# mitsuba-renderer/enoki

Measured on AMD Instinct MI355X. Metric: Gelem/s + %HBM-roofline, 64M-elt DiffArray backward(), 1/2/4/8 MI355X, higher is better.
Workload: dtype f32; 1 GPU; cfg3b: DiffArray<HIPArray<float>> y=hsum(sin(a*x+b)), a=gather(A,idx), b=gather(B,idx), K=1Mi; backward() with scatter_add grads; elements_total=67108864, elements_per_gpu=67108864, table_size=1048576, world_size=1, backend=none (single process), step_replay=eager (python-driven steps: tape walk, allocator, one launch call per kernel)

## Files before the change

enoki_amd/csrc/bucketed_early.hip:

```cpp
#include "ek_bucketed.h"
#include "ek_refine.h"

#include <cstdlib>
#include <cstring>

namespace ek {

template <int Map, int Keep, typename T> struct EarlyPair {
    static __device__ __forceinline__ void apply(T u, T &val, T &kept) {
        if constexpr ((Map == EK_SIN && Keep == EK_COS) || (Map == EK_COS && Keep == EK_SIN)) {
            T sn, cs;
            SinCosOp::apply(u, sn, cs);
            val = Map == EK_SIN ? sn : cs;
            kept = Map == EK_SIN ? cs : sn;
        } else if constexpr (Map == Keep) {
            val = kept = UnaryOp<Map, T>::apply(u);
        } else {
            val = UnaryOp<Map, T>::apply(u);
            kept = UnaryOp<Keep, T>::apply(u);
        }
    }
};

#ifdef EK_EARLY_TIMING
__device__ unsigned long long g_early_timing[32];
#endif

template <typename T, int V, int Map, int Keep, bool Two>
struct EarlyBody {
    static constexpr bool Paired = sizeof(T) == 4;
    struct Step { Pack<uint16_t, 4> pi[V]; T px[V][4]; };
    const PairRec<T> *rec;
    T *tables;
    unsigned long long *dummy;
    const uint16_t *pair_idx;
    const T *x_b;
    int Bins;
    uint32_t lmask;
    T acc[4];
#ifdef EK_EARLY_TIMING
    unsigned long long tacc[5] = { 0, 0, 0, 0, 0 }, tlast = 0, tmark[2] = { 0, 0 };
    __device__ __forceinline__ void mark(int k) { tmark[k] = __builtin_readcyclecounter(); }
    __device__ __forceinline__ void stamp(int k) { const unsigned long long now = __builtin_readcyclecounter(); tacc[k] += now - tlast; tlast = now; }
#endif

    __device__ __forceinline__ void values(uint32_t l, T x, T &sum, T &v0, T &v1) const {
        const PairRec<T> r = rec[l];
        EarlyPair<Map, Keep, T>::apply(pair_value(r.a, x, r.c, Two), sum, v0);
        v1 = dev::safe_mul(x, v0);
    }
    __device__ __forceinline__ void one(size_t pos, bool on, int slot) {
        const uint32_t l = on ? (uint32_t) pair_idx[pos] & lmask : 0u;
        T sum, v0, v1;
        values(l, on ? x_b[pos] : T(0), sum, v0, v1);
        if (on) acc[slot] += sum;
        if constexpr (Paired) {
            lds_add_pair(reinterpret_cast<unsigned long long *>(tables) + l, v0, v1, on);
        } else {
            lds_add<true>(&tables[l], v0, on);
            lds_add<true>(&tables[Bins + l], v1, on);
        }
    }
    __device__ __forceinline__ void fetch(Step &s, int h, size_t pos) {
        s.pi[h] = pack_load<uint16_t, 4, true>(pair_idx + pos);
        load4<T, true>(x_b + pos, s.px[h]);
    }
    __device__ __forceinline__ void apply(const Step &s) {
        constexpr int NB = 4 * V;
        uint32_t l[NB];
        T v0[NB], v1[NB];
        if constexpr (Paired) {
            unsigned long long *tb = reinterpret_cast<unsigned long long *>(tables);
            PairRec<T> r[NB];
#ifdef EK_EARLY_TIMING
            tlast = __builtin_readcyclecounter();
            asm volatile("s_waitcnt vmcnt(3)" ::: "memory");
            stamp(0);
#endif
#pragma unroll
            for (int k = 0; k < NB; ++k) {
                l[k] = (uint32_t) s.pi[k / 4].v[k % 4] & lmask;
                r[k] = rec[l[k]];
            }
#ifdef EK_EARLY_TIMING
            asm volatile("s_waitcnt lgkmcnt(0)" ::: "memory");
            stamp(1);
#endif
            unsigned pending = 0;
#pragma unroll
            for (int k = 0; k < NB; ++k) {
                const T x = s.px[k / 4][k % 4];
                T sum;
                EarlyPair<Map, Keep, T>::apply(pair_value(r[k].a, x, r[k].c, Two), sum, v0[k]);
                v1[k] = dev::safe_mul(x, v0[k]);
                acc[k % 4] += sum;
                pending |= lds_try_add_pair(tb, dummy, l[k], v0[k], v1[k]) ? 1u << k : 0u;
            }
#ifdef EK_EARLY_TIMING
            asm volatile("s_waitcnt lgkmcnt(0)" ::: "memory");
            stamp(2);
#endif
            if (__builtin_amdgcn_ballot_w64(pending != 0)) lds_add_pair_retry<NB>(tb, l, v0, v1, pending);
#ifdef EK_EARLY_TIMING
            asm volatile("s_waitcnt lgkmcnt(0)" ::: "memory");
            stamp(3);
            tacc[4] += 1;
#endif
            return;
        }
#pragma unroll
        for (int k = 0; k < NB; ++k) {
            l[k] = (uint32_t) s.pi[k / 4].v[k % 4] & lmask;
            T sum;
            values(l[k], s.px[k / 4][k % 4], sum, v0[k], v1[k]);
            acc[k % 4] += sum;
        }
        if constexpr (!Paired) {
            lds_add_batch<T, NB>(tables, l, v0);
            lds_add_batch<T, NB>(tables + Bins, l, v1);
        }
    }
};



__device__ __forceinline__ unsigned long long to_fixed64(float v, double up) {
    const double d = __builtin_fma((double) v, up, 6755399441055744.0);
    return __builtin_bit_cast(unsigned long long, d) - 0x4338000000000000ull;
}

constexpr uint32_t kFixedRecBytes = 4096u * 8u;

template <int PS, int Map, int Keep, bool Two>
struct EarlyFixed {
    using T = float;
    static constexpr uint32_t Page = 1u << PS, LX = Page / 4, PW = 64 / LX;
    struct Step { Pack<uint16_t, 4> pi; T px[4]; };
    const unsigned char *lds;
    const uint16_t *pair_idx;
    const T *x_b;
    uint32_t m8;
    double up0, up1;
    long long iacc;

    __device__ __forceinline__ void fetch(Step &s, size_t pos) {
#ifdef EK_FX_DIAG_IDXPAIR
        const uint32_t lane = threadIdx.x & 63u, even = (lane / (2 * LX)) * 2 * LX + lane % LX;
        const uint32_t page = (uint32_t) (pos >> PS), pa = (uint32_t) __shfl((int) page, (int) even, 64);
        const size_t posl = ((size_t) (pa & ~1u) << PS) + (((lane / LX) & 1u) << PS) + (pos & (Page - 1u));
        s.pi = pack_load<uint16_t, 4, true>(pair_idx + posl);
#else
        s.pi = pack_load<uint16_t, 4, true>(pair_idx + pos);
#endif
        load4<T, true>(x_b + pos, s.px);
    }
    struct Recs { uint32_t a8[4]; PairRec<T> r[4]; };
    __device__ __forceinline__ void lookup(const Step &s, Recs &o) const {
        uint32_t w[2];
        __builtin_memcpy(w, &s.pi, 8);
        o.a8[0] = (w[0] << 3) & m8; o.a8[1] = (w[0] >> 13) & m8;
        o.a8[2] = (w[1] << 3) & m8; o.a8[3] = (w[1] >> 13) & m8;
#pragma unroll
        for (int k = 0; k < 4; ++k) o.r[k] = *reinterpret_cast<const PairRec<T> *>(lds + o.a8[k]);
#ifdef EK_FX_DIAG_NOLOOKUP
#pragma unroll
        for (int k = 0; k < 4; ++k) o.r[k] = PairRec<T>{ __uint_as_float(o.a8[k] | 0x3f000000u), T(0.25) };
#endif
    }
    template <bool Masked>
    __device__ __forceinline__ void apply(const Step &s, const Recs &rc, int rem) {
        const uint32_t *a8 = rc.a8;
        const PairRec<T> *r = rc.r;
        int batch = 0;
#pragma unroll
        for (int k = 0; k < 4; ++k) {
            const T x = s.px[k];
            const T u = pair_value(r[k].a, x, r[k].c, Two);
            T sn = T(0), cs = T(0);
#ifdef EK_FX_DIAG_NOSINCOS
            sn = u; cs = u * T(0.5);
#else
            dev::sincos_f32<Map == EK_SIN || Keep == EK_SIN, Map == EK_COS || Keep == EK_COS, true>(u, sn, cs);
#endif
            const T sum = Map == EK_SIN ? sn : cs;
            T v0 = Keep == EK_SIN ? sn : cs;
            int q = dev::cvt_sat_i32(sum * 268435456.0f);
            if constexpr (Masked) {
                const bool on = k < rem;
                q = on ? q : 0;
                v0 = on ? v0 : T(0);
            }
            batch += q;
            const T v1 = dev::safe_mul(x, v0);
            unsigned long long *p = reinterpret_cast<unsigned long long *>(const_cast<unsigned char *>(lds) + kFixedRecBytes + a8[k]);
            unsigned long long *p1 = reinterpret_cast<unsigned long long *>(const_cast<unsigned char *>(lds) + 2 * kFixedRecBytes + a8[k]);
#ifdef EK_FX_DIAG_NOADDS
            batch += (int) (to_fixed64(v0, up0) >> 20) + (int) (to_fixed64(v1, up1) >> 20) + (int) (size_t) p;
#else
            (void) __hip_atomic_fetch_add(p, to_fixed64(v0, up0), __ATOMIC_RELAXED, __HIP_MEMORY_SCOPE_WORKGROUP);
            (void) __hip_atomic_fetch_add(p1, to_fixed64(v1, up1), __ATOMIC_RELAXED, __HIP_MEMORY_SCOPE_WORKGROUP);
#endif
        }
        iacc += (long long) batch;
    }
    __device__ __forceinline__ void flush() { }
};

template <int PS, typename Body>
__device__ __forceinline__ void walk_pages_dynamic(const BucketLists &bl, const PieceRange &r, Body &body, uint32_t *s_next) {
    using Step = typename Body::Step;
    constexpr uint32_t LX = Body::LX, PW = Body::PW, Page = Body::Page;
    const uint32_t lane = threadIdx.x & 63u, gw = lane / LX, i = lane % LX, wave = threadIdx.x >> 6;
    const uint32_t nfull = r.f1 - r.f0, nparts = r.p1 - r.p0, total = nfull + nparts, nb = (total + PW - 1u) / PW;
    auto grab = [&]() -> uint32_t {
        uint32_t v = 0;
        if (lane == 0) v = __hip_atomic_fetch_add(s_next, 1u, __ATOMIC_RELAXED, __HIP_MEMORY_SCOPE_WORKGROUP);
        return v;
    };
    auto entry = [&](uint32_t b) -> uint32_t {
        const uint32_t q = b * PW + gw;
        const uint32_t *a = q < nfull ? bl.glist_full + r.f0 + q : q < total ? bl.glist_part + r.p0 + (q - nfull) : bl.base;
        return __builtin_nontemporal_load(a);
    };
    auto place = [&](uint32_t b, uint32_t ev, size_t &pos, int &rem) {
        const uint32_t q = b * PW + gw;
        const uint32_t page = q < nfull ? ev : q < total ? ev >> 6 : 0u;
        const uint32_t count = q < nfull ? Page : q < total ? (ev & 63u) + 1u : 0u;
        pos = ((size_t) page << PS) + 4u * i;
        rem = (int) count - (int) (4u * i);
    };
    uint32_t id0 = wave, id1 = wave + kBucketWaves, id2 = wave + 2 * kBucketWaves, id3 = wave + 3 * kBucketWaves, id4 = wave + 4 * kBucketWaves;
    if (id0 >= nb) return;
    uint32_t evA = entry(id0), evB = entry(id1);
    const uint32_t ev2 = entry(id2);
    Step st0, st1, st2, st3;
    typename Body::Recs r0, r1;
    size_t pos;
    int rem0, rem1, rem2, rem3 = 0;
    place(id0, evA, pos, rem0);
    body.fetch(st0, pos);
    place(id1, evB, pos, rem1);
    body.fetch(st1, pos);
    evB = entry(id3);
    place(id2, ev2, pos, rem2);
    body.fetch(st2, pos);
    body.lookup(st0, r0);
    auto phase = [&](const Step &cur, const Step &next, Step &last, const typename Body::Recs &rc, typename Body::Recs &rn, int remc, int &reml,
                     uint32_t &ev_new, uint32_t ev_old) -> bool {
        const uint32_t g5 = grab();
        ev_new = entry(id4);
        place(id3, ev_old, pos, reml);
        body.fetch(last, pos);
        body.lookup(next, rn);
        if (__builtin_amdgcn_ballot_w64(remc < 4)) body.template apply<true>(cur, rc, remc);
        else body.template apply<false>(cur, rc, 4);
        id0 = id1; id1 = id2; id2 = id3; id3 = id4; id4 = (uint32_t) __builtin_amdgcn_readfirstlane((int) g5);
        return id0 < nb;
    };
    while (true) {
        if (!phase(st0, st1, st3, r0, r1, rem0, rem3, evA, evB)) break;
        if (!phase(st1, st2, st0, r1, r0, rem1, rem0, evB, evA)) break;
        if (!phase(st2, st3, st1, r0, r1, rem2, rem1, evA, evB)) break;
        if (!phase(st3, st0, st2, r1, r0, rem3, rem2, evB, evA)) break;
    }
    body.flush();
}


struct RefinedStream {
    const float *x;
    const uint16_t *hdr;
    const uint32_t *tiles;
    uint32_t cap_tiles;
};
struct NoRefinedStream { };
template <bool Refined> using RefinedArg = std::conditional_t<Refined, RefinedStream, NoRefinedStream>;

template <int Map, int Keep, bool Two>
struct EarlyRefined {
    using T = float;
    struct Step { uint32_t h; T px[4]; };
    struct Recs { uint32_t a8; PairRec<T> r; };
    const unsigned char *lds;
    uint32_t m8;
    double up0, up1;
    long long iacc;

    __device__ __forceinline__ void lookup(const Step &s, Recs &o) const {
        o.a8 = (s.h << 3) & m8;
        o.r = *reinterpret_cast<const PairRec<T> *>(lds + o.a8);
    }
    __device__ __forceinline__ void apply(const Step &s, const Recs &rc) {
        const int count = (int) (s.h >> kRefineEntryBits);
        int batch = 0;
        unsigned long long s0 = 0ull, s1 = 0ull;
#pragma unroll
        for (int k = 0; k < 4; ++k) {
            const T x = s.px[k];
            const T u = pair_value(rc.r.a, x, rc.r.c, Two);
            T sn = T(0), cs = T(0);
            dev::sincos_f32<Map == EK_SIN || Keep == EK_SIN, Map == EK_COS || Keep == EK_COS, true>(u, sn, cs);
            const T sum = Map == EK_SIN ? sn : cs;
            T v0 = Keep == EK_SIN ? sn : cs;
            int q = dev::cvt_sat_i32(sum * 268435456.0f);
            const bool on = k < count;
            q = on ? q : 0;
            v0 = on ? v0 : T(0);
            batch += q;
            const T v1 = dev::safe_mul(x, v0);
            s0 += to_fixed64(v0, up0);
            s1 += to_fixed64(v1, up1);
        }
        unsigned long long *p = reinterpret_cast<unsigned long long *>(const_cast<unsigned char *>(lds) + kFixedRecBytes + rc.a8);
        unsigned long long *p1 = reinterpret_cast<unsigned long long *>(const_cast<unsigned char *>(lds) + 2 * kFixedRecBytes + rc.a8);
        (void) __hip_atomic_fetch_add(p, s0, __ATOMIC_RELAXED, __HIP_MEMORY_SCOPE_WORKGROUP);
        (void) __hip_atomic_fetch_add(p1, s1, __ATOMIC_RELAXED, __HIP_MEMORY_SCOPE_WORKGROUP);
        iacc += (long long) batch;
    }
};

template <typename Body>
__device__ __forceinline__ void walk_tiles_dynamic(const RefinedStream &rs, uint32_t t0, uint32_t t1, Body &body, uint32_t *s_next) {
    using Step = typename Body::Step;
    constexpr uint32_t R = kRefineR;
    static_assert(R % 4 == 0);
    const uint32_t lane = threadIdx.x & 63u, wave = threadIdx.x >> 6, nt = t1 - t0;
    uint32_t tile0 = wave, tile1 = wave + kBucketWaves;
    if (tile0 >= nt) return;
    auto fetch = [&](Step &s, uint32_t tile, uint32_t g) {
        const size_t slot = ((size_t) (t0 + tile) * R + g) * 64u + lane;
        s.h = (uint32_t) __builtin_nontemporal_load(rs.hdr + slot);
        load4<float, true>(rs.x + slot * 4u, s.px);
    };
    Step st0, st1, st2, st3;
    typename Body::Recs r0, r1;
    fetch(st0, tile0, 0);
    fetch(st1, tile0, 1);
    fetch(st2, tile0, 2);
    body.lookup(st0, r0);
    while (true) {
        uint32_t g2 = 0;
        if (lane == 0) g2 = __hip_atomic_fetch_add(s_next, 1u, __ATOMIC_RELAXED, __HIP_MEMORY_SCOPE_WORKGROUP);
        const uint32_t tnext = tile1 < nt ? tile1 : tile0;
        auto phase = [&](uint32_t g, const Step &cur, const Step &next, Step &last, const typename Body::Recs &rc, typename Body::Recs &rn) {
            const uint32_t gf = g + 3u;
            fetch(last, gf < R ? tile0 : tnext, gf & (R - 1u));
            body.lookup(next, rn);
            body.apply(cur, rc);
        };
        for (uint32_t g = 0; g < R; g += 4) {
            phase(g, st0, st1, st3, r0, r1);
            phase(g + 1, st1, st2, st0, r1, r0);
            phase(g + 2, st2, st3, st1, r0, r1);
            phase(g + 3, st3, st0, st2, r1, r0);
        }
        tile0 = tile1;
        tile1 = (uint32_t) __builtin_amdgcn_readfirstlane((int) g2);
        if (tile0 >= nt) break;
    }
}

__device__ __forceinline__ void bucket_finish_fixed_begin(long long iblock , float fblock , float *__restrict__ partials,
                                                          uint32_t *__restrict__ ticket, uint32_t *s_last_fixed ) {
    unsigned long long *ipartials = reinterpret_cast<unsigned long long *>(partials);
    uint32_t *fpartials = reinterpret_cast<uint32_t *>(ipartials + gridDim.x);
    if (threadIdx.x == 0) {
        __hip_atomic_store(ipartials + blockIdx.x, (unsigned long long) iblock, __ATOMIC_RELAXED, __HIP_MEMORY_SCOPE_AGENT);
        __hip_atomic_store(fpartials + blockIdx.x, __float_as_uint(fblock), __ATOMIC_RELAXED, __HIP_MEMORY_SCOPE_AGENT);
#ifdef EK_EARLY_TIMING
        const unsigned long long t_tk = __builtin_readcyclecounter();
#endif
        *s_last_fixed = finish_ticket(ticket) ? 1u : 0u;
#ifdef EK_EARLY_TIMING
        const unsigned long long dt_tk = __builtin_readcyclecounter() - t_tk;
        atomicAdd(&g_early_timing[24], dt_tk); atomicMax(&g_early_timing[25], dt_tk);
#endif
    }
}
__device__ __forceinline__ void bucket_finish_fixed_end(const uint32_t *s_last_fixed , float *__restrict__ partials,
                                                        uint32_t *__restrict__ ticket, float *__restrict__ out, const uint32_t *__restrict__ active,
                                                        size_t n, int map_op, float *wave_part, long long *wave_ipart, uint32_t *__restrict__ counters,
                                                        float zero_u) {
    unsigned long long *ipartials = reinterpret_cast<unsigned long long *>(partials);
    uint32_t *fpartials = reinterpret_cast<uint32_t *>(ipartials + gridDim.x);
    __syncthreads();
    if (!*s_last_fixed) return;
    if (counters) {
        for (unsigned k = threadIdx.x; k < kPgTotalsWords + 4u; k += blockDim.x) counters[k] = 0u;
        for (unsigned k = kPgMetaBase + kPgMetaAccumRep + threadIdx.x; k < kPgMetaBase + kPgMetaAccumRepEnd; k += blockDim.x) counters[k] = 0u;
    }
    long long iv = 0;
    float fv = 0.f;
    for (unsigned i = threadIdx.x; i < gridDim.x; i += blockDim.x) {
        iv += (long long) __hip_atomic_load(ipartials + i, __ATOMIC_RELAXED, __HIP_MEMORY_SCOPE_AGENT);
        fv += __uint_as_float(__hip_atomic_load(fpartials + i, __ATOMIC_RELAXED, __HIP_MEMORY_SCOPE_AGENT));
    }
#pragma unroll
    for (int d = 32; d >= 1; d >>= 1) { iv += bucket_shfl_down(iv, d); fv += bucket_shfl_down(fv, d); }
    __syncthreads();
    if ((threadIdx.x & 63) == 0) { wave_ipart[threadIdx.x >> 6] = iv; wave_part[threadIdx.x >> 6] = fv; }
    __syncthreads();
    if (threadIdx.x < 64) {
        iv = threadIdx.x < blockDim.x / 64 ? wave_ipart[threadIdx.x] : 0ll;
        fv = threadIdx.x < blockDim.x / 64 ? wave_part[threadIdx.x] : 0.f;
#pragma unroll
        for (int d = 8; d >= 1; d >>= 1) { iv += bucket_shfl_down(iv, d); fv += bucket_shfl_down(fv, d); }
        if (threadIdx.x == 0) {
            const float r = (float) iv * 3.7252902984619140625e-9f  + fv;
            out[0] = bucket_dropped_lanes<float, EK_HSUM>(r, active ? n - (size_t) active[0] : 0, active && active[1], map_op, zero_u);
            finish_ticket_reset(ticket);
        }
    }
}

template <typename T, int V, int PS, bool Fixed, bool Two, bool Refined>
__device__ __forceinline__ void bucket_pair_forward_adjoint(T *__restrict__ partials, T *__restrict__ table_partials,
                                                            const T *__restrict__ table_a, const T *__restrict__ table_c, const T addend,
                                                            size_t table_size, int flip_a, int flip_c,
                                                            const uint16_t *__restrict__ pair_idx, const T *__restrict__ x_b,
                                                            const BucketLists &bl, int map_op, int keep_op, int shift,
                                                            const BucketFinish<T> &fin, const int zero_op, const T zero_u,
                                                            const uint32_t *__restrict__ xmax_bits, int S0,
                                                            uint32_t *__restrict__ piece_mode, const RefinedArg<Refined> &refined,
                                                            T *__restrict__ direct1) {
    static_assert(!Refined || (Fixed && sizeof(T) == 4), "the refined stream feeds the fixed-point walk only");
    extern __shared__ __align__(16) unsigned char lds_dynamic[];
    __shared__ __align__(16) unsigned char lds_static[Fixed ? 3 * kFixedRecBytes : 16];
    unsigned char *lds_raw = Fixed ? lds_static : lds_dynamic;
    const int Bins = 1 << shift;
    PairRec<T> *rec = reinterpret_cast<PairRec<T> *>(lds_raw);
    T *tables = Fixed ? reinterpret_cast<T *>(lds_raw + kFixedRecBytes) : reinterpret_cast<T *>(rec + Bins);
    __shared__ T wave_part[kBucketWaves];
    __shared__ unsigned long long s_dummy;
    __shared__ uint32_t s_next;
    __shared__ uint32_t s_guard[2];
    __shared__ long long wave_ipart[Fixed ? kBucketWaves : 1];
    __shared__ uint32_t s_last_fixed;
    constexpr bool Paired = sizeof(T) == 4;
    int bucket;
    PieceRange range;
#ifdef EK_EARLY_TIMING
    const unsigned long long t_entry = __builtin_readcyclecounter();
#endif
    [[maybe_unused]] uint32_t xm_early = 0, tile_first = 0, tile_end = 0;
    if constexpr (Refined) {
        tile_first = min(refined.tiles[blockIdx.x], refined.cap_tiles);
        tile_end = min(refined.tiles[blockIdx.x + 1], refined.cap_tiles);
    }
    if constexpr (Fixed) {
        xm_early = xmax_bits[0];
        if (threadIdx.x == 0) { s_next = (Refined ? 2u : 5u) * kBucketWaves; s_guard[0] = 0u; s_guard[1] = 0u; }
    }
    if (!bucket_piece<PS>(bl, bucket, range)) {
        if constexpr (Fixed) {
            bucket_finish_fixed_begin(0ll, T(0), partials, fin.ticket, &s_last_fixed);
            bucket_finish_fixed_end(&s_last_fixed, partials, fin.ticket, fin.out, fin.active, fin.n, zero_op, wave_part, wave_ipart, fin.counters, zero_u);
        }
        else bucket_finish<T, EK_HSUM>(T(0), partials, fin.ticket, fin.out, fin.active, fin.n, zero_op, wave_part, fin.counters, zero_u);
        return;
    }
#ifdef EK_EARLY_TIMING
    const unsigned long long t_piece = __builtin_readcyclecounter();
#endif
#ifdef EK_EARLY_TIMING
    unsigned long long fx_t[6] = { 0, 0, 0, 0, 0, 0 };
    fx_t[0] = __builtin_readcyclecounter();
#endif
    [[maybe_unused]] uint32_t slice_max[2] = { 0u, 0u };
    stage_pair_slice<T, true>(rec, tables, table_a, table_c, addend, (size_t) bucket * Bins, table_size, Bins, flip_a, flip_c, Fixed ? slice_max : nullptr);
    if constexpr (Fixed) {
        for (int j = threadIdx.x; j < 2 * 4096; j += kBucketThreads) reinterpret_cast<unsigned long long *>(tables)[j] = 0ull;
    }
    if constexpr (Fixed) {
        uint32_t am = slice_max[0], cm = slice_max[1];
#pragma unroll
        for (int d = 32; d >= 1; d >>= 1) { am = max(am, (uint32_t) __shfl_xor((int) am, d, 64)); cm = max(cm, (uint32_t) __shfl_xor((int) cm, d, 64)); }
        if ((threadIdx.x & 63) == 0) { atomicMax(&s_guard[0], am); atomicMax(&s_guard[1], cm); }
    }
    __syncthreads();
    T v = T(0);
#ifdef EK_EARLY_TIMING
    unsigned long long t_walk_end = 0;
#endif
    auto run = [&](auto body) {
        body.rec = rec; body.tables = tables; body.pair_idx = pair_idx; body.x_b = x_b; body.Bins = Bins;
        body.lmask = (uint32_t) Bins - 1u; body.dummy = &s_dummy;
#pragma unroll
        for (int k = 0; k < 4; ++k) body.acc[k] = T(0);
#ifdef EK_EARLY_TIMING
        const unsigned long long t_begin = __builtin_readcyclecounter();
#endif
        walk_piece<PS, V>(bl, range, body);
#ifdef EK_EARLY_TIMING
        if ((threadIdx.x & 255) == 0) {
            const unsigned long long t_end = __builtin_readcyclecounter();
            for (int k = 0; k < 5; ++k) atomicAdd(&g_early_timing[k], body.tacc[k]);
            atomicAdd(&g_early_timing[5], t_end - t_begin);
            atomicAdd(&g_early_timing[6], 1ull);
            atomicAdd(&g_early_timing[7], body.tmark[0] - t_begin);
            atomicAdd(&g_early_timing[8], body.tmark[1] - body.tmark[0]);
            atomicAdd(&g_early_timing[9], t_end - body.tmark[1]);
            atomicAdd(&g_early_timing[10], t_piece - t_entry);
            atomicAdd(&g_early_timing[11], t_begin - t_piece);
            atomicMax(&g_early_timing[12], t_end - t_begin);
            t_walk_end = t_end;
        }
#endif
        v = (body.acc[0] + body.acc[1]) + (body.acc[2] + body.acc[3]);
    };
    [[maybe_unused]] bool locks = !Fixed, single = false;
    [[maybe_unused]] long long iv = 0;
    [[maybe_unused]] FixedScale fixed0{}, fixed1{};
    if constexpr (Fixed) {
        const uint32_t xm = (uint32_t) __builtin_amdgcn_readfirstlane((int) xm_early);
        const uint32_t E = xm >> 23;
        locks = E >= 255u || (E < (uint32_t) S0 + 1u && xm != 0u);
        const uint32_t am = s_guard[0], cm = s_guard[1];
        const float ubound = __uint_as_float(am) * __uint_as_float(xm) + __uint_as_float(cm);
        const size_t piece_pages = (size_t) (range.f1 - range.f0) + (range.p1 - range.p0);
        if (am >= 0x7F800000u || cm >= 0x7F800000u || !(ubound < 1.0e18f) || (piece_pages << PS) >> (62 - S0)) locks = true;
        single = range.pieces == 1u;
        if (threadIdx.x == 0) piece_mode[blockIdx.x] = (locks || single) ? 1u : 0u;
        if (!locks) {
            fixed0 = fixed_scale(S0, xm, false);
            fixed1 = fixed_scale(S0, xm, true);
            auto run_fixed = [&](auto body) {
                body.lds = lds_raw; body.pair_idx = pair_idx; body.x_b = x_b;
                asm volatile("v_mov_b32 %0, %1" : "=v"(body.m8) : "s"(((uint32_t) Bins - 1u) << 3));
                body.up0 = fixed0.upd; body.up1 = fixed1.upd; body.iacc = 0;
#ifdef EK_EARLY_TIMING
                fx_t[1] = __builtin_readcyclecounter();
#endif
                walk_pages_dynamic<PS>(bl, range, body, &s_next);
#ifdef EK_EARLY_TIMING
                fx_t[2] = __builtin_readcyclecounter();
#endif
                iv = body.iacc;
            };
            [[maybe_unused]] auto run_refined = [&](auto body) {
                if constexpr (Refined) {
                    body.lds = lds_raw;
                    asm volatile("v_mov_b32 %0, %1" : "=v"(body.m8) : "s"(((uint32_t) Bins - 1u) << 3));
                    body.up0 = fixed0.upd; body.up1 = fixed1.upd; body.iacc = 0;
                    walk_tiles_dynamic(refined, (uint32_t) __builtin_amdgcn_readfirstlane((int) tile_first),
                                       (uint32_t) __builtin_amdgcn_readfirstlane((int) tile_end), body, &s_next);
                    iv = body.iacc;
                }
            };
            if constexpr (Refined) {
                if (map_op == EK_SIN && keep_op == EK_COS) run_refined(EarlyRefined<EK_SIN, EK_COS, Two>{});
                else if (map_op == EK_COS && keep_op == EK_SIN) run_refined(EarlyRefined<EK_COS, EK_SIN, Two>{});
                else if (map_op == EK_SIN) run_refined(EarlyRefined<EK_SIN, EK_SIN, Two>{});
                else run_refined(EarlyRefined<EK_COS, EK_COS, Two>{});
            } else
            if (map_op == EK_SIN && keep_op == EK_COS) run_fixed(EarlyFixed<PS, EK_SIN, EK_COS, Two>{});
            else if (map_op == EK_COS && keep_op == EK_SIN) run_fixed(EarlyFixed<PS, EK_COS, EK_SIN, Two>{});
            else if (map_op == EK_SIN) run_fixed(EarlyFixed<PS, EK_SIN, EK_SIN, Two>{});
            else run_fixed(EarlyFixed<PS, EK_COS, EK_COS, Two>{});
        }
    }
    if (locks) {
#define EK_EARLY_CASE(M, K) else if (map_op == M && keep_op == K) run(EarlyBody<T, V, M, K, Two>{});
        if (map_op == EK_SIN && keep_op == EK_COS) run(EarlyBody<T, V, EK_SIN, EK_COS, Two>{});
        EK_EARLY_CASE(EK_COS, EK_SIN) EK_EARLY_CASE(EK_LOG, EK_RCP) EK_EARLY_CASE(EK_SQRT, EK_RSQRT) EK_EARLY_CASE(EK_RCP, EK_RCP_SQR)
        EK_EARLY_CASE(EK_RSQRT, EK_RSQRT_CUBE) EK_EARLY_CASE(EK_SIN, EK_SIN) EK_EARLY_CASE(EK_COS, EK_COS)
        EK_EARLY_CASE(EK_EXP, EK_EXP) EK_EARLY_CASE(EK_SQRT, EK_SQRT) EK_EARLY_CASE(EK_RCP, EK_RCP) EK_EARLY_CASE(EK_RSQRT, EK_RSQRT)
        EK_EARLY_CASE(EK_LOG, EK_LOG) EK_EARLY_CASE(EK_ABS, EK_ABS) EK_EARLY_CASE(EK_NEG, EK_NEG)
#undef EK_EARLY_CASE
    }
#pragma unroll
    for (int d = 32; d >= 1; d >>= 1) v += bucket_shfl_down(v, d);
    const int lane = threadIdx.x & 63, wave = threadIdx.x >> 6;
    if constexpr (Fixed) {
#pragma unroll
        for (int d = 32; d >= 1; d >>= 1) iv += bucket_shfl_down(iv, d);
        if (lane == 0) wave_ipart[wave] = iv;
    }
    if (lane == 0) wave_part[wave] = v;
    __syncthreads();
#ifdef EK_EARLY_TIMING
    fx_t[3] = __builtin_readcyclecounter();
#endif
    if (threadIdx.x < 64) {
        v = threadIdx.x < kBucketWaves ? wave_part[threadIdx.x] : T(0);
#pragma unroll
        for (int d = 8; d >= 1; d >>= 1) v += bucket_shfl_down(v, d);
        if constexpr (Fixed) {
            iv = threadIdx.x < kBucketWaves ? wave_ipart[threadIdx.x] : 0ll;
#pragma unroll
            for (int d = 8; d >= 1; d >>= 1) iv += bucket_shfl_down(iv, d);
        }
    }
    if constexpr (Fixed) bucket_finish_fixed_begin(iv, v, partials, fin.ticket, &s_last_fixed);
    [[maybe_unused]] bool direct = false;
    if constexpr (Fixed) direct = direct1 != nullptr;
    if (direct) {
        if constexpr (Fixed) {
            const size_t first = (size_t) bucket * Bins;
            const int lim = first < table_size ? (int) (table_size - first < (size_t) Bins ? table_size - first : (size_t) Bins) : 0;
            const uint32_t xm_fold = (uint32_t) __builtin_amdgcn_readfirstlane((int) xm_early);
#pragma unroll
            for (int c = 0; c < 2; ++c) {
                float *plane = (c ? direct1 : table_partials) + first;
                const float back = fixed_scale(S0, xm_fold, c == 1).back;
                if (!locks) {
                    const long long *sums = reinterpret_cast<const long long *>(lds_raw + (c + 1) * kFixedRecBytes);
                    const float own = c ? fixed1.back : fixed0.back;
                    for (int j = threadIdx.x; j < lim; j += kBucketThreads) {
                        const float fsum = (float) sums[j] * own;
                        const float v = (float) (long long) 0ull * back + fsum;
                        plane[j] = 0.f + v;
                    }
                } else {
                    for (int j = threadIdx.x; j < lim; j += kBucketThreads) {
                        const float fsum = tables[2 * j + c];
                        const float v = (float) (long long) 0ull * back + fsum;
                        plane[j] = 0.f + v;
                    }
                }
            }
        }
    } else
#pragma unroll
    for (int c = 0; c < 2; ++c) {
        T *out = table_partials + ((size_t) c * gridDim.x + blockIdx.x) * Bins;
        if constexpr (Fixed) {
            long long *out64 = reinterpret_cast<long long *>(table_partials) + ((size_t) c * gridDim.x + blockIdx.x) * Bins;
            if (!locks && single) {
                const long long *sums = reinterpret_cast<const long long *>(lds_raw + (c + 1) * kFixedRecBytes);
                const float back = c ? fixed1.back : fixed0.back;
                T *outf = reinterpret_cast<T *>(out64);
                for (int j = threadIdx.x; j < Bins; j += kBucketThreads) outf[j] = (float) sums[j] * back;
            } else if (!locks) {
                const long long *sums = reinterpret_cast<const long long *>(lds_raw + (c + 1) * kFixedRecBytes);
                for (int j = threadIdx.x; j < Bins; j += kBucketThreads) out64[j] = sums[j];
            } else {
                T *outf = reinterpret_cast<T *>(out64);
                for (int j = threadIdx.x; j < Bins; j += kBucketThreads) outf[j] = tables[2 * j + c];
            }
        } else {
            for (int j = threadIdx.x; j < Bins; j += kBucketThreads) out[j] = Paired ? tables[2 * j + c] : tables[c * Bins + j];
        }
    }
#ifdef EK_EARLY_TIMING
    if (threadIdx.x == 0) {
        asm volatile("s_waitcnt vmcnt(0)" ::: "memory");
        const unsigned long long t_out = __builtin_readcyclecounter();
        atomicAdd(&g_early_timing[13], t_out - t_walk_end);
        atomicAdd(&g_early_timing[14], t_out - t_entry);
        atomicMax(&g_early_timing[15], t_out - t_entry);
    }
#endif
#ifdef EK_EARLY_TIMING
    if constexpr (Fixed) {
        asm volatile("s_waitcnt vmcnt(0)" ::: "memory");
        fx_t[4] = __builtin_readcyclecounter();
    }
#endif
    if constexpr (Fixed) bucket_finish_fixed_end(&s_last_fixed, partials, fin.ticket, fin.out, fin.active, fin.n, zero_op, wave_part, wave_ipart, fin.counters, zero_u);
    else bucket_finish<T, EK_HSUM>(v, partials, fin.ticket, fin.out, fin.active, fin.n, zero_op, wave_part, fin.counters, zero_u);
#ifdef EK_EARLY_TIMING
    if constexpr (Fixed) {
        if (threadIdx.x == 0 && fx_t[1]) {
            fx_t[5] = __builtin_readcyclecounter();
            atomicAdd(&g_early_timing[16], fx_t[0] - t_entry);
            atomicAdd(&g_early_timing[17], fx_t[1] - fx_t[0]);
            atomicAdd(&g_early_timing[18], fx_t[2] - fx_t[1]);
            atomicAdd(&g_early_timing[19], fx_t[3] - fx_t[2]);
            atomicAdd(&g_early_timing[20], fx_t[4] - fx_t[3]);
            atomicAdd(&g_early_timing[21], fx_t[5] - fx_t[4]);
            atomicAdd(&g_early_timing[22], 1ull);
            atomicMax(&g_early_timing[23], fx_t[5] - t_entry);
        }
    }
#endif
}

template <typename T, int V, int PS, bool Fixed, bool Two, bool Refined>
__global__ __launch_bounds__(kBucketThreads) void k_bucket_pair_forward_adjoint(T *__restrict__ partials, T *__restrict__ table_partials,
                                                                                const T *__restrict__ table_a,
                                                                                const T *__restrict__ table_c, size_t table_size,
                                                                                int flip_a, int flip_c,
                                                                                const uint16_t *__restrict__ pair_idx,
                                                                                const T *__restrict__ x_b, BucketLists bl,
                                                                                int map_op, int keep_op, int shift, BucketFinish<T> fin,
                                                                                const uint32_t *__restrict__ xmax_bits, int S0,
                                                                                uint32_t *__restrict__ piece_mode, RefinedArg<Refined> refined,
                                                                                T *__restrict__ direct1) {
    bucket_pair_forward_adjoint<T, V, PS, Fixed, Two, Refined>(partials, table_partials, table_a, table_c, T(-0.0), table_size, flip_a, flip_c, pair_idx,
                                                               x_b, bl, map_op, keep_op, shift, fin, fin.zero_op, T(0), xmax_bits, S0, piece_mode, refined,
                                                               direct1);
}

template <typename T, int V, int PS, bool Fixed, bool Two, bool Refined>
__global__ __launch_bounds__(kBucketThreads) void k_bucket_pair_forward_adjoint_scalar(T *__restrict__ partials, T *__restrict__ table_partials,
                                                                                       const T *__restrict__ table_a, T addend,
                                                                                       size_t table_size, int flips,
                                                                                       const uint16_t *__restrict__ pair_idx,
                                                                                       const T *__restrict__ x_b, BucketLists bl,
                                                                                       int map_op, int keep_op, int shift, BucketFinish<T> fin,
                                                                                       const uint32_t *__restrict__ xmax_bits, int S0,
                                                                                       uint32_t *__restrict__ piece_mode, RefinedArg<Refined> refined) {
    bucket_pair_forward_adjoint<T, V, PS, Fixed, Two, Refined>(partials, table_partials, table_a, nullptr, addend, table_size, flips & 1, flips & 2, pair_idx,
                                                               x_b, bl, map_op, keep_op, shift, fin, map_op, fin.zero_u, xmax_bits, S0, piece_mode, refined,
                                                               nullptr );
}

static int partition_one_piece(BucketPartition *p) {
    if (!p->piece_prefix || p->n_buckets <= 0) { p->one_piece_state = -1; return EK_OK; }
    std::vector<uint32_t> prefix((size_t) p->n_buckets + 1, 0u);
    EK_HIP_CHECK(hipMemcpyAsync(prefix.data(), p->piece_prefix, prefix.size() * sizeof(uint32_t), hipMemcpyDeviceToHost, ctx().stream));
    EK_HIP_CHECK(hipStreamSynchronize(ctx().stream));
    bool one = true;
    for (int k = 0; k < p->n_buckets; ++k) one = one && prefix[(size_t) k + 1] - prefix[(size_t) k] == 1u;
    p->one_piece_state = one ? 1 : -1;
    return EK_OK;
}

template <typename T>
int bucketed_forward_adjoint_launch(Bucketed *b, void *out, int map_op, int keep_op) {
    Context &c = ctx();
    const size_t Bins = b->bins();
    size_t lds = Bins * (sizeof(PairRec<T>) + 2 * sizeof(T));
    constexpr int VV = 1;
    const int flip_a = b->flip_a(), flip_c = b->flip_c(), two = b->two_roundings();
    const bool bounded = (map_op == EK_SIN || map_op == EK_COS) && (keep_op == EK_SIN || keep_op == EK_COS);
    const bool fixed = sizeof(T) == 4 && early_fixed_enabled() && bounded && b->page_shift != 0 && b->active && Bins * 8 <= kFixedRecBytes;
    const size_t slot = fixed ? sizeof(long long) : sizeof(T);
    const bool scalar = b->scalar_addend;
    const bool eager = refuse_while_capturing_quiet() == EK_OK;
    bool direct = false;
    if constexpr (sizeof(T) == 4) {
        const int mode = c.tuning.direct_tables;
        if (fixed && eager && !scalar && !b->addend_broadcast && b->part && b->stands_on_kept &&
            (mode == 2 || (mode == 1 && b->table_size >= kDirectTablesMinEntries))) {
            if (b->part->one_piece_state == 0)
                if (int rc = partition_one_piece(b->part)) return rc;
            direct = b->part->one_piece_state == 1;
        }
    }
    if (direct) {
        const size_t plane_bytes = (std::max<size_t>(b->table_size, 1) * sizeof(T) + 15) & ~(size_t) 15;
        if (!b->direct[0])
            if (int rc = ek_hip_malloc(plane_bytes + (size_t) b->max_pieces * sizeof(uint32_t), &b->direct[0])) return rc;
        if (!b->direct[1])
            if (int rc = ek_hip_malloc(plane_bytes, &b->direct[1])) return rc;
        b->direct_modes = static_cast<char *>(b->direct[0]) + plane_bytes;
    } else if (!b->early)
        if (int rc = ek_hip_malloc((size_t) 2 * b->max_pieces * Bins * slot + (fixed ? (size_t) b->max_pieces * sizeof(uint32_t) : 0), &b->early)) return rc;
    const size_t piece_bound = 2 * (b->n / std::max<size_t>(1, b->max_pieces - (size_t) b->n_buckets)) + 65536;
    const int S0 = std::min(fixed_shift_for(piece_bound), 48);
    uint32_t *modes = direct ? (uint32_t *) b->direct_modes
                    : fixed ? reinterpret_cast<uint32_t *>(static_cast<char *>(b->early) + (size_t) 2 * b->max_pieces * Bins * slot) : nullptr;
    T *plane0 = direct ? (T *) b->direct[0] : (T *) b->early, *direct1 = direct ? (T *) b->direct[1] : nullptr;
    if (fixed && eager && b->part && b->stands_on_kept && b->part->refine_state == 0 && Bins <= ((size_t) 1 << kRefineEntryBits))
        if (int rc = partition_refine(b->part)) return rc;
    const bool use_refined = fixed && eager && b->part && b->part->refine_state == 1;
    const uint32_t *xmax = fixed ? b->active + (kPgMetaResultXmax - kPgMetaResult) : nullptr;
    auto go = [&](auto kernel, auto kernel_scalar, auto kernel_refined, auto kernel_scalar_refined) -> int {
        if (int rc = scalar ? allow_big_lds(kernel_scalar, lds) : allow_big_lds(kernel, lds)) return rc;
        const BucketFinish<T> fin = b->template finish<T>(out, map_op);
        if constexpr (!std::is_same_v<decltype(kernel_refined), std::nullptr_t>) {
            const BucketPartition *p = b->part;
            if (use_refined && scalar) {
                if (fin.zero_op != map_op || b->table_c) return fail(EK_ERR_INVALID, "bucketed_forward_adjoint_launch(): inconsistent scalar-addend object");
                hipLaunchKernelGGL(kernel_scalar_refined, dim3(b->max_pieces), dim3(kBucketThreads), lds, c.stream,
                                   (T *) b->reduce_partials, (T *) b->early, (const T *) b->table_a, b->template addend<T>(), b->table_size,
                                   flip_a | (flip_c << 1), (const uint16_t *) b->pair_idx, (const T *) b->x_b, b->lists(), map_op, keep_op, b->shift,
                                   fin, xmax, S0, modes, RefinedStream{ p->refined_x, p->refined_hdr, p->refined_tiles, p->refined_cap_tiles });
                return EK_OK;
            }
            if (use_refined) {
                hipLaunchKernelGGL(kernel_refined, dim3(b->max_pieces), dim3(kBucketThreads), lds, c.stream,
                                   (T *) b->reduce_partials, plane0, (const T *) b->table_a, (const T *) b->table_c, b->table_size,
                                   flip_a, flip_c, (const uint16_t *) b->pair_idx, (const T *) b->x_b, b->lists(), map_op, keep_op, b->shift,
                                   fin, xmax, S0, modes, RefinedStream{ p->refined_x, p->refined_hdr, p->refined_tiles, p->refined_cap_tiles }, direct1);
                return EK_OK;
            }
        }
        if (scalar) {
            if (fin.zero_op != map_op || b->table_c) return fail(EK_ERR_INVALID, "bucketed_forward_adjoint_launch(): inconsistent scalar-addend object");
            hipLaunchKernelGGL(kernel_scalar, dim3(b->max_pieces), dim3(kBucketThreads), lds, c.stream,
                               (T *) b->reduce_partials, (T *) b->early, (const T *) b->table_a, b->template addend<T>(), b->table_size,
                               flip_a | (flip_c << 1), (const uint16_t *) b->pair_idx, (const T *) b->x_b, b->lists(), map_op, keep_op, b->shift,
                               fin, xmax, S0, modes, NoRefinedStream{});
        } else {
            hipLaunchKernelGGL(kernel, dim3(b->max_pieces), dim3(kBucketThreads), lds, c.stream,
                               (T *) b->reduce_partials, plane0, (const T *) b->table_a, (const T *) b->table_c, b->table_size,
                               flip_a, flip_c, (const uint16_t *) b->pair_idx, (const T *) b->x_b, b->lists(), map_op, keep_op, b->shift,
                               fin, xmax, S0, modes, NoRefinedStream{}, direct1);
        }
        return EK_OK;
    };
#define EK_PAIR(PSV, FIXED, TWO) go(k_bucket_pair_forward_adjoint<T, VV, PSV, FIXED, TWO, false>, k_bucket_pair_forward_adjoint_scalar<T, VV, PSV, FIXED, TWO, false>, nullptr, nullptr)
#define EK_PAIR_FIXED(PSV, TWO) go(k_bucket_pair_forward_adjoint<T, VV, PSV, true, TWO, false>, k_bucket_pair_forward_adjoint_scalar<T, VV, PSV, true, TWO, false>, \
                                   k_bucket_pair_forward_adjoint<T, VV, PSV, true, TWO, true>, k_bucket_pair_forward_adjoint_scalar<T, VV, PSV, true, TWO, true>)
    int rc;
    if constexpr (sizeof(T) == 8) {
        rc = two ? EK_PAIR(0, false, true) : EK_PAIR(0, false, false);
    } else {
        if (fixed) lds = 0;
#define EK_GO(PSV) (fixed ? (two ? EK_PAIR_FIXED(PSV, true) : EK_PAIR_FIXED(PSV, false)) : (two ? EK_PAIR(PSV, false, true) : EK_PAIR(PSV, false, false)))
        rc = b->page_shift == 6 ? EK_GO(6) : EK_GO(5);
#undef EK_GO
    }
#undef EK_PAIR
#undef EK_PAIR_FIXED
    if (rc) return rc;
    const size_t stream_bytes = use_refined ? 18u * (b->n / 4u + 3u * std::min(b->n, b->table_size) / 8u) : b->n * (sizeof(uint16_t) + sizeof(T));
    EK_LAUNCH_CHECK("bucket_pair_fma_reduce_adjoint", b->n,
                    stream_bytes + (b->table_c ? 2 : 1) * b->table_size * sizeof(T) +
                    (direct ? 2 * b->table_size * sizeof(T) : (size_t) 2 * b->max_pieces * Bins * slot));
    b->launched_reducing();
    b->early_direct = direct;
    b->early_fixed = fixed;
    b->early_S0 = S0;
    b->early_modes = modes;
    b->has_early = true;
    b->early_op = keep_op;
    if (!b->ticket) {
        hipLaunchKernelGGL((k_bucket_reduce_final<T, EK_HSUM>), dim3(1), dim3(256), 0, c.stream, (T *) out, (const T *) b->reduce_partials,
                           b->max_pieces, b->masked_ptr(), b->n, map_op, b->template dropped_u<T>());
        EK_LAUNCH_CHECK("reduce_stage2", (size_t) b->max_pieces, (size_t) b->max_pieces * sizeof(T) + sizeof(T));
    }
    return EK_OK;
}

template int bucketed_forward_adjoint_launch<float>(Bucketed *, void *, int, int);
template int bucketed_forward_adjoint_launch<double>(Bucketed *, void *, int, int);

}

#ifdef EK_EARLY_TIMING
extern "C" EK_API int ek_hip_debug_early_timing(unsigned long long *out8) {
    (void) hipDeviceSynchronize();
    (void) hipMemcpyFromSymbol(out8, HIP_SYMBOL(ek::g_early_timing), 32 * sizeof(unsigned long long));
    unsigned long long zero[32] = {};
    (void) hipMemcpyToSymbol(HIP_SYMBOL(ek::g_early_timing), zero, sizeof(zero));
    return EK_OK;
}
#endif
```

Before: 839.3 Gelem/s.

## Stream finished bucket table bins to global memory while tile walk progresses

Adds a per-workgroup frontier: each wave publishes the table entry it is currently at (the refined stream is sorted by entry), and the minimum over the waves marks bins that no wave can touch again. A wave that advances the shared done marker writes those completed fixed-point sums out early, overlapping the table writeback with the walk instead of doing it all after. The tail writes only the remaining bins. This adds LDS atomics, DPP reductions and write work inside the hot loop, and it is only correct if entries really are monotonic per wave.

```diff
diff --git a/enoki_amd/csrc/bucketed_early.hip b/enoki_amd/csrc/bucketed_early.hip
--- a/enoki_amd/csrc/bucketed_early.hip
+++ b/enoki_amd/csrc/bucketed_early.hip
@@ -1,5 +1,6 @@
 #include "ek_bucketed.h"
 #include "ek_refine.h"
+#include "ek_frontier.h"
 
 #include <cstdlib>
 #include <cstring>
@@ -319,14 +320,15 @@
     }
 };
 
-template <typename Body>
-__device__ __forceinline__ void walk_tiles_dynamic(const RefinedStream &rs, uint32_t t0, uint32_t t1, Body &body, uint32_t *s_next) {
+template <typename Body, typename Frontier>
+__device__ __forceinline__ void walk_tiles_dynamic(const RefinedStream &rs, uint32_t t0, uint32_t t1, Body &body, uint32_t *s_next,
+                                                   const Frontier &frontier) {
     using Step = typename Body::Step;
     constexpr uint32_t R = kRefineR;
     static_assert(R % 4 == 0);
     const uint32_t lane = threadIdx.x & 63u, wave = threadIdx.x >> 6, nt = t1 - t0;
     uint32_t tile0 = wave, tile1 = wave + kBucketWaves;
-    if (tile0 >= nt) return;
+    if (tile0 >= nt) { frontier.leave(); return; }
     auto fetch = [&](Step &s, uint32_t tile, uint32_t g) {
         const size_t slot = ((size_t) (t0 + tile) * R + g) * 64u + lane;
         s.h = (uint32_t) __builtin_nontemporal_load(rs.hdr + slot);
@@ -338,6 +340,7 @@
     fetch(st1, tile0, 1);
     fetch(st2, tile0, 2);
     body.lookup(st0, r0);
+    typename Frontier::Look look = frontier.publish_and_look(st0.h & ((1u << kRefineEntryBits) - 1u));
     while (true) {
         uint32_t g2 = 0;
         if (lane == 0) g2 = __hip_atomic_fetch_add(s_next, 1u, __ATOMIC_RELAXED, __HIP_MEMORY_SCOPE_WORKGROUP);
@@ -357,8 +360,54 @@
         tile0 = tile1;
         tile1 = (uint32_t) __builtin_amdgcn_readfirstlane((int) g2);
         if (tile0 >= nt) break;
-    }
-}
+        frontier.claim(look, kFrontierMinClaim);
+        look = frontier.publish_and_look(st0.h & ((1u << kRefineEntryBits) - 1u));
+    }
+    frontier.leave();
+}
+
+#ifndef EK_PROGRESSIVE_TABLES
+#define EK_PROGRESSIVE_TABLES 1
+#endif
+template <typename Write>
+struct TileFrontier {
+    uint32_t *front, *done;
+    uint32_t bins;
+    const Write &write;
+    struct Look { uint32_t f, d; };
+    static_assert(kBucketWaves == 16, "the minimum over the waves is taken inside one DPP row of 16 lanes");
+
+    __device__ __forceinline__ Look ask() const {
+        Look l;
+        l.f = __hip_atomic_load(front + (threadIdx.x & (kBucketWaves - 1u)), __ATOMIC_RELAXED, __HIP_MEMORY_SCOPE_WORKGROUP);
+        l.d = __hip_atomic_load(done, __ATOMIC_RELAXED, __HIP_MEMORY_SCOPE_WORKGROUP);
+        asm volatile("" ::: "memory");
+        return l;
+    }
+    __device__ __forceinline__ Look publish_and_look(uint32_t entry) const {
+        if constexpr (!EK_PROGRESSIVE_TABLES) return Look{ 0u, 0u };
+        asm volatile("" ::: "memory");
+        if ((threadIdx.x & 63u) == 0u) __hip_atomic_store(front + (threadIdx.x >> 6), entry, __ATOMIC_RELAXED, __HIP_MEMORY_SCOPE_WORKGROUP);
+        return ask();
+    }
+    __device__ __forceinline__ void claim(const Look &l, uint32_t least) const {
+        if constexpr (!EK_PROGRESSIVE_TABLES) return;
+        uint32_t m = l.f;
+        m = min(m, (uint32_t) __builtin_amdgcn_update_dpp((int) m, (int) m, 0x128 , 0xf, 0xf, false));
+        m = min(m, (uint32_t) __builtin_amdgcn_update_dpp((int) m, (int) m, 0x124 , 0xf, 0xf, false));
+        m = min(m, (uint32_t) __builtin_amdgcn_update_dpp((int) m, (int) m, 0x122 , 0xf, 0xf, false));
+        m = min(m, (uint32_t) __builtin_amdgcn_update_dpp((int) m, (int) m, 0x121 , 0xf, 0xf, false));
+        const uint32_t fmin = (uint32_t) __builtin_amdgcn_readfirstlane((int) m), seen = (uint32_t) __builtin_amdgcn_readfirstlane((int) l.d);
+        const uint32_t target = frontier_target(fmin, seen, least);
+        if (target == seen) return;
+        uint32_t old = 0;
+        if ((threadIdx.x & 63u) == 0u) old = __hip_atomic_fetch_max(done, target, __ATOMIC_RELAXED, __HIP_MEMORY_SCOPE_WORKGROUP);
+        old = (uint32_t) __builtin_amdgcn_readfirstlane((int) old);
+        if (frontier_owns(old, target)) write(std::integral_constant<int, 4>{}, (int) old, (int) target, (int) (threadIdx.x & 63u), 64);
+    }
+    __device__ __forceinline__ void leave() const { claim(publish_and_look(bins), kFrontierRound); }
+};
+
 
 __device__ __forceinline__ void bucket_finish_fixed_begin(long long iblock , float fblock , float *__restrict__ partials,
                                                           uint32_t *__restrict__ ticket, uint32_t *s_last_fixed ) {
@@ -436,6 +485,7 @@
     __shared__ uint32_t s_guard[2];
     __shared__ long long wave_ipart[Fixed ? kBucketWaves : 1];
     __shared__ uint32_t s_last_fixed;
+    __shared__ uint32_t s_front[kBucketWaves], s_done;
     constexpr bool Paired = sizeof(T) == 4;
     int bucket;
     PieceRange range;
@@ -450,6 +500,10 @@
     if constexpr (Fixed) {
         xm_early = xmax_bits[0];
         if (threadIdx.x == 0) { s_next = (Refined ? 2u : 5u) * kBucketWaves; s_guard[0] = 0u; s_guard[1] = 0u; }
+        if constexpr (Refined) {
+            if (threadIdx.x < kBucketWaves) s_front[threadIdx.x] = 0u;
+            if (threadIdx.x == 0) s_done = 0u;
+        }
     }
     if (!bucket_piece<PS>(bl, bucket, range)) {
         if constexpr (Fixed) {
@@ -511,8 +565,58 @@
     [[maybe_unused]] bool locks = !Fixed, single = false;
     [[maybe_unused]] long long iv = 0;
     [[maybe_unused]] FixedScale fixed0{}, fixed1{};
+    [[maybe_unused]] bool direct = false;
+    if constexpr (Fixed) direct = direct1 != nullptr;
+    [[maybe_unused]] auto write_fixed = [&](auto in_flight, int e0, int e1, int first_thread, int stride) {
+        constexpr int U = decltype(in_flight)::value;
+        auto sweep = [&](const long long *sums, int hi, auto &&store) {
+            if constexpr (U == 1) {
+                for (int j = e0 + first_thread; j < hi; j += stride) store(j, sums[j]);
+            } else {
+                for (int j = e0 + first_thread; j < hi; j += U * stride) {
+                    long long s[U];
+#pragma unroll
+                    for (int k = 0; k < U; ++k) s[k] = j + k * stride < hi ? sums[j + k * stride] : 0ll;
+#pragma unroll
+                    for (int k = 0; k < U; ++k)
+                        if (j + k * stride < hi) store(j + k * stride, s[k]);
+                }
+            }
+        };
+        if constexpr (Fixed) {
+            if (direct) {
+                const size_t first = (size_t) bucket * Bins;
+                const int lim = first < table_size ? (int) (table_size - first < (size_t) Bins ? table_size - first : (size_t) Bins) : 0;
+                const uint32_t xm_fold = (uint32_t) __builtin_amdgcn_readfirstlane((int) xm_early);
+#pragma unroll
+                for (int c = 0; c < 2; ++c) {
+                    float *plane = (c ? direct1 : table_partials) + first;
+                    const float back = fixed_scale(S0, xm_fold, c == 1).back;
+                    const float own = c ? fixed1.back : fixed0.back;
+                    sweep(reinterpret_cast<const long long *>(lds_raw + (c + 1) * kFixedRecBytes), e1 < lim ? e1 : lim, [&](int j, long long sum) {
+                        const float fsum = (float) sum * own;
+                        const float v = (float) (long long) 0ull * back + fsum;
+                        plane[j] = 0.f + v;
+                    });
+                }
+            } else {
+#pragma unroll
+                for (int c = 0; c < 2; ++c) {
+                    long long *out64 = reinterpret_cast<long long *>(table_partials) + ((size_t) c * gridDim.x + blockIdx.x) * Bins;
+                    const long long *sums = reinterpret_cast<const long long *>(lds_raw + (c + 1) * kFixedRecBytes);
+                    if (single) {
+                        const float back = c ? fixed1.back : fixed0.back;
+                        T *outf = reinterpret_cast<T *>(out64);
+                        sweep(sums, e1, [&](int j, long long sum) { outf[j] = (float) sum * back; });
+                    } else {
+                        sweep(sums, e1, [&](int j, long long sum) { out64[j] = sum; });
+                    }
+                }
+            }
+        }
+    };
     if constexpr (Fixed) {
-        const uint32_t xm = (uint32_t) __builtin_amdgcn_readfirstlane((int) xm_early);
+        const uint32_t xm =(uint32_t) __builtin_amdgcn_readfirstlane((int) xm_early);
         const uint32_t E = xm >> 23;
         locks = E >= 255u || (E < (uint32_t) S0 + 1u && xm != 0u);
         const uint32_t am = s_guard[0], cm = s_guard[1];
@@ -542,8 +646,15 @@
                     body.lds = lds_raw;
                     asm volatile("v_mov_b32 %0, %1" : "=v"(body.m8) : "s"(((uint32_t) Bins - 1u) << 3));
                     body.up0 = fixed0.upd; body.up1 = fixed1.upd; body.iacc = 0;
+#ifdef EK_EARLY_TIMING
+                    fx_t[1] = __builtin_readcyclecounter();
+#endif
+                    const TileFrontier<decltype(write_fixed)> frontier{ s_front, &s_done, (uint32_t) Bins, write_fixed };
                     walk_tiles_dynamic(refined, (uint32_t) __builtin_amdgcn_readfirstlane((int) tile_first),
-                                       (uint32_t) __builtin_amdgcn_readfirstlane((int) tile_end), body, &s_next);
+                                       (uint32_t) __builtin_amdgcn_readfirstlane((int) tile_end), body, &s_next, frontier);
+#ifdef EK_EARLY_TIMING
+                    fx_t[2] = __builtin_readcyclecounter();
+#endif
                     iv = body.iacc;
                 }
             };
@@ -592,26 +703,23 @@
         }
     }
     if constexpr (Fixed) bucket_finish_fixed_begin(iv, v, partials, fin.ticket, &s_last_fixed);
-    [[maybe_unused]] bool direct = false;
-    if constexpr (Fixed) direct = direct1 != nullptr;
-    if (direct) {
-        if constexpr (Fixed) {
-            const size_t first = (size_t) bucket * Bins;
-            const int lim = first < table_size ? (int) (table_size - first < (size_t) Bins ? table_size - first : (size_t) Bins) : 0;
-            const uint32_t xm_fold = (uint32_t) __builtin_amdgcn_readfirstlane((int) xm_early);
-#pragma unroll
-            for (int c = 0; c < 2; ++c) {
-                float *plane = (c ? direct1 : table_partials) + first;
-                const float back = fixed_scale(S0, xm_fold, c == 1).back;
-                if (!locks) {
-                    const long long *sums = reinterpret_cast<const long long *>(lds_raw + (c + 1) * kFixedRecBytes);
-                    const float own = c ? fixed1.back : fixed0.back;
-                    for (int j = threadIdx.x; j < lim; j += kBucketThreads) {
-                        const float fsum = (float) sums[j] * own;
-                        const float v = (float) (long long) 0ull * back + fsum;
-                        plane[j] = 0.f + v;
-                    }
-                } else {
+    if constexpr (Fixed) {
+        if (!locks) {
+            int written = 0;
+            if constexpr (Refined) written = (int) s_done;
+            write_fixed(std::integral_constant<int, 1>{}, written, Bins, (int) threadIdx.x, kBucketThreads);
+        }
+    }
+    if (locks) {
+        if (direct) {
+            if constexpr (Fixed) {
+                const size_t first = (size_t) bucket * Bins;
+                const int lim = first < table_size ? (int) (table_size - first < (size_t) Bins ? table_size - first : (size_t) Bins) : 0;
+                const uint32_t xm_fold = (uint32_t) __builtin_amdgcn_readfirstlane((int) xm_early);
+#pragma unroll
+                for (int c = 0; c < 2; ++c) {
+                    float *plane = (c ? direct1 : table_partials) + first;
+                    const float back = fixed_scale(S0, xm_fold, c == 1).back;
                     for (int j = threadIdx.x; j < lim; j += kBucketThreads) {
                         const float fsum = tables[2 * j + c];
                         const float v = (float) (long long) 0ull * back + fsum;
@@ -619,27 +727,16 @@
                     }
                 }
             }
-        }
-    } else
-#pragma unroll
-    for (int c = 0; c < 2; ++c) {
-        T *out = table_partials + ((size_t) c * gridDim.x + blockIdx.x) * Bins;
-        if constexpr (Fixed) {
-            long long *out64 = reinterpret_cast<long long *>(table_partials) + ((size_t) c * gridDim.x + blockIdx.x) * Bins;
-            if (!locks && single) {
-                const long long *sums = reinterpret_cast<const long long *>(lds_raw + (c + 1) * kFixedRecBytes);
-                const float back = c ? fixed1.back : fixed0.back;
-                T *outf = reinterpret_cast<T *>(out64);
-                for (int j = threadIdx.x; j < Bins; j += kBucketThreads) outf[j] = (float) sums[j] * back;
-            } else if (!locks) {
-                const long long *sums = reinterpret_cast<const long long *>(lds_raw + (c + 1) * kFixedRecBytes);
-                for (int j = threadIdx.x; j < Bins; j += kBucketThreads) out64[j] = sums[j];
+        } else
+#pragma unroll
+        for (int c = 0; c < 2; ++c) {
+            T *out = table_partials + ((size_t) c * gridDim.x + blockIdx.x) * Bins;
+            if constexpr (Fixed) {
+                T *outf = reinterpret_cast<T *>(reinterpret_cast<long long *>(table_partials) + ((size_t) c * gridDim.x + blockIdx.x) * Bins);
+                for (int j = threadIdx.x; j < Bins; j += kBucketThreads) outf[j] = tables[2 * j + c];
             } else {
-                T *outf = reinterpret_cast<T *>(out64);
-                for (int j = threadIdx.x; j < Bins; j += kBucketThreads) outf[j] = tables[2 * j + c];
+                for (int j = threadIdx.x; j < Bins; j += kBucketThreads) out[j] = Paired ? tables[2 * j + c] : tables[c * Bins + j];
             }
-        } else {
-            for (int j = threadIdx.x; j < Bins; j += kBucketThreads) out[j] = Paired ? tables[2 * j + c] : tables[c * Bins + j];
         }
     }
 #ifdef EK_EARLY_TIMING
diff --git a/enoki_amd/csrc/ek_frontier.h b/enoki_amd/csrc/ek_frontier.h
--- /dev/null
+++ b/enoki_amd/csrc/ek_frontier.h
@@ -0,0 +1,34 @@
+#pragma once
+#include <cstdint>
+
+#if defined(__HIPCC__) || defined(__CUDACC__)
+#define EK_FRONTIER_HD __host__ __device__
+#else
+#define EK_FRONTIER_HD
+#endif
+
+namespace ek {
+
+constexpr uint32_t kFrontierRound = 64;
+constexpr uint32_t kFrontierMinClaim = 256;
+constexpr uint32_t kFrontierMaxClaim = 512;
+static_assert(kFrontierMinClaim % kFrontierRound == 0 && kFrontierMaxClaim % kFrontierRound == 0 && kFrontierMinClaim <= kFrontierMaxClaim,
+              "claims are whole trips");
+
+EK_FRONTIER_HD inline uint32_t frontier_min(const uint32_t *front, uint32_t waves) {
+    uint32_t f = front[0];
+    for (uint32_t w = 1; w < waves; ++w) f = front[w] < f ? front[w] : f;
+    return f;
+}
+
+EK_FRONTIER_HD inline uint32_t frontier_target(uint32_t fmin, uint32_t done, uint32_t least) {
+    uint32_t target = fmin & ~(kFrontierRound - 1u);
+    if (target > done + kFrontierMaxClaim) target = done + kFrontierMaxClaim;
+    return target >= done + least ? target : done;
+}
+
+EK_FRONTIER_HD inline bool frontier_owns(uint32_t old, uint32_t target) { return old < target; }
+
+EK_FRONTIER_HD inline uint32_t frontier_remainder(uint32_t done, uint32_t bins) { return done < bins ? bins - done : 0u; }
+
+}
```

Measured after the change: 813.0 Gelem/s. 0.969x the previous value.
